# opendilab/DI-engine

Hardware: NVIDIA H100
Metric: learner transitions/sec (GAE+ppo_error fwd+bwd, T=128 x B=4096 per GPU) (higher is better)
Workload: dtype f32

## Files before the change

### di-engine_b200/csrc/gae_tile.cuh

```cuda
#pragma once
#include "common.cuh"

namespace b200rl {

template <int ID, int COUNT>
__device__ __forceinline__ void named_bar_sync() {
    asm volatile("bar.sync %0, %1;" ::"n"(ID), "n"(COUNT) : "memory");
}
template <int ID, int COUNT>
__device__ __forceinline__ void named_bar_arrive() {
    asm volatile("bar.arrive %0, %1;" ::"n"(ID), "n"(COUNT) : "memory");
}
template <int COUNT>
__device__ __forceinline__ void chunk_arrive(int k) {
    if (k == 0) named_bar_arrive<1, COUNT>();
    else if (k == 1) named_bar_arrive<2, COUNT>();
    else if (k == 2) named_bar_arrive<3, COUNT>();
    else named_bar_arrive<4, COUNT>();
}
__device__ __forceinline__ void scanned_arrive(int k) {
    if (k == 0) named_bar_arrive<5, 64>();
    else if (k == 1) named_bar_arrive<6, 64>();
    else if (k == 2) named_bar_arrive<7, 64>();
    else named_bar_arrive<8, 64>();
// ... 97 lines not shown
                        const long long c = c0 + cc;
                        if (r >= 0 && c < C) {
                            const long long off = (lo + r) * C + c;
                            const long long aoff = (lo + r) * Caux + c / A;
                            float nvv = next_value[off];
                            if (vscale != 0.f) nvv = fmul(nvv, vscale);
                            const float dnn = done ? done[aoff] : 0.f;
                            const float tff = traj ? traj[aoff] : dnn;
                            if (done) {
                                const float mm = fmul(nvv, fsub(1.f, dnn));
                                if (mask_inplace && dnn != 0.f) next_value[off] = mm;
                                nvv = mm;
                            }
                            const float vvv = vscale != 0.f ? fmul(value[off], vscale) : value[off];
                            s_d[k][rr][cc] = fsub(fadd(reward[aoff], fmul(gamma, nvv)), vvv);
                            s_f[k][rr][cc] = fmul(gl, fsub(1.f, tff));
                        }
                    }
                    chunk_arrive<NTHREADS>(k);
                }
            }
        } else {
            const int cc = threadIdx.x;
            const bool lane_ok = cc < TC && c0 + cc < C;
#pragma unroll 1
            for (int k = 0; k < GAE_NCHUNK; ++k) {
                chunk_wait<NTHREADS>(k);
                const int rtop = rows - 1 - k * GAE_CH;
                if (lane_ok && rtop >= 0) {
                    if (rtop >= GAE_CH - 1) {
                        float d[GAE_CH], f[GAE_CH];
#pragma unroll
                        for (int j = 0; j < GAE_CH; ++j) {
                            d[j] = s_d[k][j][cc];
                            f[j] = s_f[k][j][cc];
                        }
#pragma unroll
                        for (int j = 0; j < GAE_CH; ++j) {
                            carry = fadd(d[j], fmul(f[j], carry));
                            s_d[k][j][cc] = carry;
                        }
                    } else {
                        for (int j = 0; j <= rtop; ++j) {
                            carry = fadd(s_d[k][j][cc], fmul(s_f[k][j][cc], carry));
                            s_d[k][j][cc] = carry;
                        }
                    }
                }
                scanned_arrive(k);
            }
        }
        if (!is_scan) {
            constexpr int NLW = NL / 32;
            const int lw = ltid >> 5, ll = ltid & 31;
#pragma unroll 1
            for (int k = 0; k < GAE_NCHUNK; ++k) {
                if (k % NLW != lw) continue;
                scanned_wait(k);
                const int rtop = rows - 1 - k * GAE_CH;
                if (VEC) {
                    constexpr int TPR = TC / 4;
                    for (int i = ll; i < GAE_CH * TPR; i += 32) {
                        const int rr = i / TPR, cq = (i % TPR) * 4;
                        const int r = rtop - rr;
                        if (r >= 0 && c0 + cq < C) {
                            const float4 a4 = *reinterpret_cast<const float4*>(&s_d[k][rr][cq]);
                            stg_stream4(reinterpret_cast<float4*>(adv + (lo + r) * C + c0 + cq), a4);
                        }
                    }
                } else {
                    for (int i = ll; i < GAE_CH * TC; i += 32) {
                        const int rr = i / TC, cc = i % TC;
                        const int r = rtop - rr;
                        if (r >= 0 && c0 + cc < C) adv[(lo + r) * C + c0 + cc] = s_d[k][rr][cc];
                    }
                }
                on_chunk_done((T - hi) / GAE_CH + k, rtop >= 0);
            }
        }
        if (lo > 0) __syncthreads();
    }
}

}
```

### di-engine_b200/csrc/policy.cu

```cuda
#include <math.h>

#include "../../include/b200rl.h"
#include "policy_stats.cuh"

namespace b200rl {

constexpr int GS_NT = 1024;
constexpr int GS_MAX_T = 24576;

template <int VN>
__global__ void __launch_bounds__(GS_NT) gae_seq_kernel(const float* __restrict__ value, float* __restrict__ next_value,
                                                       const float* __restrict__ reward, const float* __restrict__ done,
                                                       const float* __restrict__ traj, float* __restrict__ adv, int T,
                                                       float gamma, float gl, int mask_inplace, RetArgs ra) {
    pdl_prologue();
    extern __shared__ float s_seq[];
    float* s_d = s_seq;
    float* s_f = s_seq + T;
    __shared__ int s_nseg;
    __shared__ int s_cnt[GS_NT / 32];
    const int tid = threadIdx.x;
    const float vs = ra.vscale;
    float mu = 0.f, sigma = 1.f;
    if constexpr (VN == VN_POPART) {
        mu = *ra.mu;
        sigma = *ra.sigma;
    }
    for (int t = tid; t < T; t += GS_NT) {
        const float v = vn_decode<VN>(value[t], vs);
        float nv = vn_decode<VN>(next_value[t], vs);
        float r = reward[t];
        if constexpr (VN == VN_POPART) r = __fdiv_rn(fsub(r, mu), sigma);
        const float d = done ? done[t] : 0.f;
        const float tf = traj ? traj[t] : d;
        if (done) {
            nv = fmul(nv, fsub(1.f, d));
            if (VN == VN_PPO && mask_inplace && d != 0.f) next_value[t] = nv;
        }
        s_d[t] = fsub(fadd(r, fmul(gamma, nv)), v);
        s_f[t] = fmul(gl, fsub(1.f, tf));
    }
    __syncthreads();
    const int strip = (T + GS_NT - 1) / GS_NT;
    const int t0 = tid * strip, t1 = min(T, t0 + strip);
    int mine = 0;
    for (int t = t0; t < t1; ++t) mine += (s_f[t] == 0.f || t == T - 1) ? 1 : 0;
    int incl = mine;
    const int lane = tid & 31, wid = tid >> 5;
#pragma unroll
    for (int o = 1; o < 32; o <<= 1) {
        const int n = __shfl_up_sync(0xffffffffu, incl, o);
        if (lane >= o) incl += n;
    }
    if (lane == 31) s_cnt[wid] = incl;
    __syncthreads();
    if (wid == 0) {
        int w = s_cnt[lane];
#pragma unroll
        for (int o = 1; o < 32; o <<= 1) {
            const int n = __shfl_up_sync(0xffffffffu, w, o);
            if (lane >= o) w += n;
        }
        s_cnt[lane] = w;
        if (lane == 31) s_nseg = w;
    }
    __syncthreads();
    const int base = incl - mine + (wid ? s_cnt[wid - 1] : 0);
    __shared__ int s_end[GS_NT];
    const int nseg = s_nseg;
    const bool fits = nseg <= GS_NT;
    if (fits) {
        int k = base;
        for (int t = t0; t < t1; ++t)
            if (s_f[t] == 0.f || t == T - 1) s_end[k++] = t;
    }
    __syncthreads();
    if (fits) {
        if (tid < nseg) {
            const int hi = s_end[tid];
            const int lo = tid ? s_end[tid - 1] + 1 : 0;
            float carry = 0.f;
            int t = hi;
            for (; t - 15 >= lo; t -= 16) {
                float d[16], f[16];
#pragma unroll
// ... 32 lines not shown
        if (cut >= 0) atomicMax(&s_cut, cut);
        __syncthreads();
        const int c = s_cut;
        for (int t = tid; t <= c; t += GS_NT) s_d[t] = __int_as_float(0x7fc00000);
        __syncthreads();
    }
    double acc[4] = {0.0, 0.0, 0.0, 0.0}, pv[2];
    ret_pivots<VN>(vs, vn_decode<VN>(ld_after_wait(value), vs), s_d[0], pv);
    for (int t = tid; t < T; t += GS_NT) {
        const float a = s_d[t];
        adv[t] = a;
        moments_add(acc[2], acc[3], a, pv[1]);
        if (ra.ret_unnorm || ra.value_out || ra.ret_out || ra.stats) {
            float ru, vo, ro;
            moments_add(acc[0], acc[1], ret_encode<VN>(vs, vn_decode<VN>(value[t], vs), a, ru, vo, ro), pv[0]);
            if (ra.ret_unnorm) ra.ret_unnorm[t] = ru;
            if (ra.value_out) ra.value_out[t] = vo;
            if (ra.ret_out) ra.ret_out[t] = ro;
        }
    }
    if (ra.stats || ra.adv_stats) {
        double tot[4];
        if (stats_grid_join<4, GS_NT>(acc, tot, nullptr, nullptr)) write_ret_stats<VN>(ra, tot, pv, (double)T);
    }
}

template <int VN, bool VEC>
__global__ void __launch_bounds__(256) returns_kernel(const float* __restrict__ value, const float* __restrict__ adv,
                                                      long long n, RetArgs ra, double* __restrict__ ws_part,
                                                      unsigned int* __restrict__ ws_join) {
    pdl_prologue();
    const float vs = ra.vscale;
    double acc[4] = {0.0, 0.0, 0.0, 0.0}, pv[2];
    const long long stride = (long long)gridDim.x * 256;
    long long i = (long long)blockIdx.x * 256 + threadIdx.x;
    if (VEC) {
        const long long n4 = n >> 2;
        const float4* v4 = reinterpret_cast<const float4*>(value);
        const float4* a4 = reinterpret_cast<const float4*>(adv);
        float4 v = make_float4(0.f, 0.f, 0.f, 0.f), a = v;
        if (i < n4) {
            v = v4[i];
            a = a4[i];
        }
        ret_pivots<VN>(vs, ret_value<VN>(ld_after_wait(value), vs), ld_after_wait(adv), pv);
        for (; i < n4; i += stride) {
            float4 ru, vo, ro;
            ret_one<VN>(vs, v.x, a.x, ru.x, vo.x, ro.x, acc, pv);
            ret_one<VN>(vs, v.y, a.y, ru.y, vo.y, ro.y, acc, pv);
            ret_one<VN>(vs, v.z, a.z, ru.z, vo.z, ro.z, acc, pv);
            ret_one<VN>(vs, v.w, a.w, ru.w, vo.w, ro.w, acc, pv);
            if (ra.ret_unnorm) reinterpret_cast<float4*>(ra.ret_unnorm)[i] = ru;
            if (ra.value_out) reinterpret_cast<float4*>(ra.value_out)[i] = vo;
            if (ra.ret_out) reinterpret_cast<float4*>(ra.ret_out)[i] = ro;
            if (i + stride < n4) {
                v = v4[i + stride];
                a = a4[i + stride];
            }
        }
    } else {
        float v = 0.f, a = 0.f;
        if (i < n) {
            v = value[i];
            a = adv[i];
        }
        ret_pivots<VN>(vs, ret_value<VN>(ld_after_wait(value), vs), ld_after_wait(adv), pv);
        for (; i < n; i += stride) {
            float ru, vo, ro;
            ret_one<VN>(vs, v, a, ru, vo, ro, acc, pv);
            if (ra.ret_unnorm) ra.ret_unnorm[i] = ru;
            if (ra.value_out) ra.value_out[i] = vo;
            if (ra.ret_out) ra.ret_out[i] = ro;
            if (i + stride < n) {
                v = value[i + stride];
                a = adv[i + stride];
            }
        }
    }
    if (!ra.stats && !ra.adv_stats) return;
    double tot[4];
    if (stats_grid_join<4, 256>(acc, tot, ws_part, ws_join)) write_ret_stats<VN>(ra, tot, pv, (double)n);
}

__global__ void __launch_bounds__(256) adv_stats_kernel(const float* __restrict__ x, long long n, float* __restrict__ out,
                                                        double* __restrict__ ws_part, unsigned int* __restrict__ ws_join) {
    pdl_prologue();
    const double p = stats_pivot(ld_after_wait(x));
    double acc[2] = {0.0, 0.0};
    for (long long i = (long long)blockIdx.x * 256 + threadIdx.x; i < n; i += (long long)gridDim.x * 256)
        moments_add(acc[0], acc[1], x[i], p);
    double tot[2];
    if (stats_grid_join<2, 256>(acc, tot, ws_part, ws_join)) write_adv_stats(out, tot[0], tot[1], p, (double)n);
}

__global__ void __launch_bounds__(256) normalize_kernel(const float* __restrict__ x, const float* __restrict__ stats,
                                                        long long n, float* __restrict__ out) {
    pdl_prologue();
    const float m = ld_after_wait(stats), d = ld_after_wait(stats + 1);
    for (long long i = (long long)blockIdx.x * 256 + threadIdx.x; i < n; i += (long long)gridDim.x * 256)
        out[i] = __fdiv_rn(fsub(x[i], m), d);
}

__global__ void __launch_bounds__(256) impala_mask_kernel(const float* __restrict__ values, const float* __restrict__ rewards,
                                                          const float* __restrict__ done, long long T, long long B,
                                                          float* __restrict__ values_out, float* __restrict__ rewards_out,
                                                          float* __restrict__ weights_out) {
    pdl_prologue();
    const long long n = (T + 1) * B;
    for (long long i = (long long)blockIdx.x * 256 + threadIdx.x; i < n; i += (long long)gridDim.x * 256) {
        const long long t = i / B;
        const float m = t >= 1 ? fsub(1.f, done[i - B]) : 1.f;
        values_out[i] = t >= 1 ? fmul(values[i], m) : values[i];
        if (t < T) {
            if (weights_out) weights_out[i] = m;
            if (rewards_out) rewards_out[i] = fmul(rewards[i], m);
        }
    }
}

enum ValueMap : int { VM_SYMLOG = 0, VM_INV_SYMLOG = 1, VM_H_INV = 2, VM_POPART_REWARD = 3 };

template <int M>
__device__ __forceinline__ float value_map(float x, float mu, float sigma) {
    if constexpr (M == VM_SYMLOG) return vn_symlog(x);
    else if constexpr (M == VM_INV_SYMLOG) return vn_inv_symlog(x);
    else if constexpr (M == VM_H_INV) return vn_h_inv(x);
    else return __fdiv_rn(fsub(x, mu), sigma);
}

template <int M>
__global__ void __launch_bounds__(256) value_map_kernel(const float* __restrict__ x0, float* __restrict__ y0,
                                                        const float* __restrict__ x1, float* __restrict__ y1, long long n,
                                                        const float* __restrict__ mu, const float* __restrict__ sigma) {
    pdl_prologue();
    float m = 0.f, sg = 1.f;
    if constexpr (M == VM_POPART_REWARD) {
        m = *mu;
        sg = *sigma;
    }
    for (long long i = (long long)blockIdx.x * 256 + threadIdx.x; i < n; i += (long long)gridDim.x * 256) {
        y0[i] = value_map<M>(x0[i], m, sg);
        if (x1) y1[i] = value_map<M>(x1[i], m, sg);
    }
}

template <int M>
__global__ void __launch_bounds__(256) value_map_bwd_kernel(const float* __restrict__ x, const float* __restrict__ g,
                                                            float* __restrict__ dx, long long n) {
    pdl_prologue();
    for (long long i = (long long)blockIdx.x * 256 + threadIdx.x; i < n; i += (long long)gridDim.x * 256) {
        const float xi = x[i], s = vn_sign(xi), gs = fmul(g[i], s);
        const float d = M == VM_SYMLOG ? __fdiv_rn(gs, fadd(fabsf(xi), 1.f)) : fmul(gs, expf(fabsf(xi)));
        dx[i] = fadd(0.f, fmul(d, s));
    }
}

}

using namespace b200rl;

namespace b200rl {
int gae_scan(const float* value, float* next_value, const float* reward, const float* done, const float* traj_flag, float* adv,
             long long T, long long C, long long A, double gamma_d, double lambda_d, int mask_next_value_inplace,
             float vscale, void* stream);
}

static double* ws_stats_part(float* ws) { return reinterpret_cast<double*>(ws + WS_CTRL_WORDS); }
static unsigned int* ws_joins(float* ws) { return reinterpret_cast<unsigned int*>(ws + WS_FX_OFF_WORDS + 48); }
static_assert(WS_CTRL_WORDS % 2 == 0 && WS_CTRL_WORDS + NUM_SMS * 8 * 4 * 2 <= WS_PARTIAL_LIMIT_WORDS,
              "the statistics rows fit the workspace's partial region");

extern "C" int b200rl_adv_stats(const float* x, long long n, float* stats2, float* workspace, size_t workspace_bytes,
                                void* stream) {
    if (!x || !stats2 || !workspace || n < 1 || workspace_bytes < WS_MIN_BYTES) return B200RL_ERR_ARG;
    long long grid = div_up(n, 256 * 8);
    if (grid > NUM_SMS * 4) grid = NUM_SMS * 4;
    if (grid < 1) grid = 1;
    return launch_k(adv_stats_kernel, (int)grid, 256, 0, (cudaStream_t)stream, x, n, stats2, ws_stats_part(workspace),
                    ws_joins(workspace));
}

extern "C" int b200rl_normalize(const float* x, const float* stats2, long long n, float* out, void* stream) {
    if (!x || !stats2 || !out || n < 0) return B200RL_ERR_ARG;
    if (n == 0) return B200RL_OK;
    long long grid = div_up(n, 256 * 4);
    if (grid > NUM_SMS * 8) grid = NUM_SMS * 8;
    return launch_k(normalize_kernel, (int)grid, 256, 0, (cudaStream_t)stream, x, stats2, n, out);
}

extern "C" int b200rl_gae_returns(const float* value, float* next_value, const float* reward, const float* done,
                                  const float* traj_flag, long long T, long long C, long long A, double gamma,
                                  double lambda_, int mask_next_value_inplace, double value_scale, float* adv,
                                  float* unnormalized_return, float* value_out, float* return_out, float* stats3,
                                  float* adv_stats2, float* workspace, size_t workspace_bytes, void* stream) {
    if (T < 1 || C < 1 || A < 1 || !value || !next_value || !reward || !adv || !workspace ||
        workspace_bytes < WS_MIN_BYTES || value_scale < 0.0)
        return B200RL_ERR_ARG;
    RetArgs ra{};
    ra.vscale = (float)value_scale;
    ra.ret_unnorm = unnormalized_return; ra.value_out = value_out; ra.ret_out = return_out; ra.stats = stats3;
    ra.adv_stats = adv_stats2;
    cudaStream_t st = (cudaStream_t)stream;
    if (C == 1 && T <= GS_MAX_T) {
        const size_t smem = (size_t)2 * T * sizeof(float);
        if (int rc = smem_opt_in<gae_seq_kernel<VN_PPO>>(smem)) return rc;
        return launch_k(gae_seq_kernel<VN_PPO>, 1, GS_NT, smem, st, value, next_value, reward, done, traj_flag, adv, (int)T,
                        (float)gamma, (float)(gamma * lambda_), mask_next_value_inplace, ra);
    }
    const bool want_epi = unnormalized_return || value_out || return_out || stats3 || adv_stats2;
    int rc = gae_scan(value, next_value, reward, done, traj_flag, adv, T, C, A, gamma, lambda_, mask_next_value_inplace,
                      (float)value_scale, stream);
    if (rc != 0 || !want_epi) return rc;
    const long long n = T * C;
    const bool vec = (n % 4 == 0) && aligned16(value) && aligned16(adv) && (!unnormalized_return || aligned16(unnormalized_return)) &&
                     (!value_out || aligned16(value_out)) && (!return_out || aligned16(return_out));
    long long grid = div_up(n, 256 * (vec ? 8 : 4));
    if (grid > NUM_SMS * 8) grid = NUM_SMS * 8;
    if (vec)
        return launch_k(returns_kernel<VN_PPO, true>, (int)grid, 256, 0, st, value, (const float*)adv, n, ra,
                        ws_stats_part(workspace), ws_joins(workspace));
    return launch_k(returns_kernel<VN_PPO, false>, (int)grid, 256, 0, st, value, (const float*)adv, n, ra,
                    ws_stats_part(workspace), ws_joins(workspace));
}

static long long map_grid(long long n) {
    long long grid = div_up(n, 256 * 4);
    if (grid > NUM_SMS * 8) grid = NUM_SMS * 8;
    return grid < 1 ? 1 : grid;
}

template <int VN>
static int launch_gae_seq(const float* value, const float* next_value, const float* reward, const float* done,
                          const float* traj_flag, float* adv, long long T, double gamma, double lambda_, const RetArgs& ra,
                          cudaStream_t st) {
    const size_t smem = (size_t)2 * T * sizeof(float);
    if (int rc = smem_opt_in<gae_seq_kernel<VN>>(smem)) return rc;
    return launch_k(gae_seq_kernel<VN>, 1, GS_NT, smem, st, value, const_cast<float*>(next_value), reward, done, traj_flag,
                    adv, (int)T, (float)gamma, (float)(gamma * lambda_), 0, ra);
}

template <int VN>
static int launch_returns(const float* value, const float* adv, long long n, const RetArgs& ra, float* workspace,
                          cudaStream_t st) {
    const bool vec = (n % 4 == 0) && aligned16(value) && aligned16(adv) && (!ra.value_out || aligned16(ra.value_out)) &&
                     (!ra.ret_out || aligned16(ra.ret_out));
    long long grid = div_up(n, 256 * (vec ? 8 : 4));
    if (grid > NUM_SMS * 8) grid = NUM_SMS * 8;
    if (vec)
        return launch_k(returns_kernel<VN, true>, (int)grid, 256, 0, st, value, adv, n, ra, ws_stats_part(workspace),
                        ws_joins(workspace));
    return launch_k(returns_kernel<VN, false>, (int)grid, 256, 0, st, value, adv, n, ra, ws_stats_part(workspace),
                    ws_joins(workspace));
}

template <int VN>
static int launch_gae_returns_tc(const float* value, const float* next_value, const float* reward, const float* done,
                                 const float* traj_flag, float* adv, long long T, long long C, double gamma, double lambda_,
                                 const RetArgs& ra, float* scratch, float* workspace, cudaStream_t st) {
    const long long n = T * C;
    const float* v = value;
    const float* nv = next_value;
    const float* r = reward;
    int rc = 0;
    if constexpr (VN == VN_RESCALE || VN == VN_SYMLOG) {
        constexpr int M = VN == VN_RESCALE ? VM_H_INV : VM_INV_SYMLOG;
        rc = launch_k(value_map_kernel<M>, (int)map_grid(n), 256, 0, st, value, scratch, next_value, scratch + n, n,
                      (const float*)nullptr, (const float*)nullptr);
        v = scratch;
        nv = scratch + n;
    } else if constexpr (VN == VN_POPART) {
        rc = launch_k(value_map_kernel<VM_POPART_REWARD>, (int)map_grid(n), 256, 0, st, reward, scratch,
                      (const float*)nullptr, (float*)nullptr, n, ra.mu, ra.sigma);
        r = scratch;
    }
    if (rc) return rc;
    rc = gae_scan(v, const_cast<float*>(nv), r, done, traj_flag, adv, T, C, 1, gamma, lambda_, 0,
                  VN == VN_BASELINE ? ra.vscale : 0.f, st);
    if (rc || !(ra.value_out || ra.ret_out || ra.stats || ra.adv_stats)) return rc;
    return launch_returns<VN>(v, adv, n, ra, workspace, st);
}

template <int VN>
static int gae_returns_norm(const float* value, const float* next_value, const float* reward, const float* done,
                            const float* traj_flag, float* adv, long long T, long long C, double gamma, double lambda_,
                            const RetArgs& ra, float* scratch, float* workspace, cudaStream_t st) {
    if (C == 1 && T <= GS_MAX_T)
        return launch_gae_seq<VN>(value, next_value, reward, done, traj_flag, adv, T, gamma, lambda_, ra, st);
    return launch_gae_returns_tc<VN>(value, next_value, reward, done, traj_flag, adv, T, C, gamma, lambda_, ra, scratch,
                                     workspace, st);
}

extern "C" int b200rl_gae_returns_norm(const float* value, const float* next_value, const float* reward, const float* done,
// ... 64 lines not shown
```

### di-engine_b200/csrc/policy_stats.cuh

```cuda
#pragma once
#include <math.h>

#include "common.cuh"

namespace b200rl {

template <class T>
__device__ __forceinline__ T warp_sum_t(T v) {
#pragma unroll
    for (int o = 16; o > 0; o >>= 1) v += __shfl_xor_sync(0xffffffffu, v, o);
    return v;
}

template <int K, int NT>
__device__ __forceinline__ void block_sum_d(double (&v)[K], double (&tot)[K]) {
    __shared__ double s_bs[K][NT / 32];
    const int lane = threadIdx.x & 31, wid = threadIdx.x >> 5;
#pragma unroll
    for (int k = 0; k < K; ++k) {
        const double r = warp_sum_t(v[k]);
        if (lane == 0) s_bs[k][wid] = r;
    }
    __syncthreads();
    if (threadIdx.x == 0) {
// ... 7 lines not shown
    __syncthreads();
}

struct RetArgs {
    float vscale;
    float* ret_unnorm;
    float* value_out;
    float* ret_out;
    float* stats;
    float* adv_stats;
    const float* mu;
    const float* sigma;
};

enum ValueNorm : int { VN_BASELINE = 0, VN_RESCALE = 1, VN_SYMLOG = 2, VN_POPART = 3, VN_PPO = 4 };

__device__ __forceinline__ float vn_sign(float x) { return (float)((0.f < x) - (x < 0.f)); }

__device__ __forceinline__ float vn_h(float x) {
    return fadd(fmul(vn_sign(x), fsub(__fsqrt_rn(fadd(fabsf(x), 1.f)), 1.f)), fmul(0.01f, x));
}
__device__ __forceinline__ float vn_h_inv(float x) {
    const float u = __fdiv_rn(fsub(__fsqrt_rn(fadd(1.f, fmul(0.04f, fadd(fadd(fabsf(x), 1.f), 0.01f)))), 1.f), 0.02f);
    return fmul(vn_sign(x), fsub(fmul(u, u), 1.f));
}
__device__ __forceinline__ float vn_symlog(float x) { return fmul(vn_sign(x), logf(fadd(fabsf(x), 1.f))); }
__device__ __forceinline__ float vn_inv_symlog(float x) { return fmul(vn_sign(x), fsub(expf(fabsf(x)), 1.f)); }

template <int VN>
__device__ __forceinline__ float vn_decode(float v, float vs) {
    if constexpr (VN == VN_PPO || VN == VN_BASELINE) return vs != 0.f ? fmul(v, vs) : v;
    else if constexpr (VN == VN_RESCALE) return vn_h_inv(v);
    else if constexpr (VN == VN_SYMLOG) return vn_inv_symlog(v);
    else return v;
}

template <int VN>
__device__ __forceinline__ float vn_encode(float v, float vs) {
    if constexpr (VN == VN_PPO || VN == VN_BASELINE) return vs != 0.f ? __fdiv_rn(v, vs) : v;
    else if constexpr (VN == VN_RESCALE) return vn_h(v);
    else if constexpr (VN == VN_SYMLOG) return vn_symlog(v);
    else return v;
}

template <int VN>
__device__ __forceinline__ float ret_encode(float vs, float v, float a, float& ru, float& vo, float& ro) {
    const float r = fadd(v, a);
    ru = r;
    vo = vn_encode<VN>(v, vs);
    ro = vn_encode<VN>(r, vs);
    return VN == VN_PPO ? r : ro;
}

__device__ __forceinline__ double stats_pivot(float x0) { return isfinite(x0) ? (double)x0 : 0.0; }

__device__ __forceinline__ float ld_after_wait(const float* p) { return __ldcg(p); }

__device__ __forceinline__ void moments_add(double& s1, double& s2, float x, double p) {
    const double d = (double)x - p;
    s1 += d;
    s2 = fma(d, d, s2);
}

template <int VN>
__device__ __forceinline__ float ret_value(float v, float vs) {
    if constexpr (VN == VN_PPO || VN == VN_BASELINE) return vn_decode<VN>(v, vs);
    else return v;
}

template <int VN>
__device__ __forceinline__ void ret_one(float vs, float v, float a, float& ru, float& vo, float& ro, double (&acc)[4],
                                        const double (&pv)[2]) {
    moments_add(acc[0], acc[1], ret_encode<VN>(vs, ret_value<VN>(v, vs), a, ru, vo, ro), pv[0]);
    moments_add(acc[2], acc[3], a, pv[1]);
}

template <int VN>
__device__ __forceinline__ void ret_pivots(float vs, float v0, float a0, double (&pv)[2]) {
    float ru, vo, ro;
    pv[0] = stats_pivot(ret_encode<VN>(vs, v0, a0, ru, vo, ro));
    pv[1] = stats_pivot(a0);
}

template <int K, int NT>
__device__ __forceinline__ bool stats_grid_join(double (&acc)[K], double (&tot)[K], double* part, unsigned int* ticket) {
    __shared__ bool s_last;
    block_sum_d<K, NT>(acc, tot);
    if (gridDim.x == 1) return threadIdx.x == 0;
    if (threadIdx.x == 0) {
#pragma unroll
        for (int k = 0; k < K; ++k) part[(size_t)blockIdx.x * K + k] = tot[k];
        __threadfence();
        s_last = atomicAdd(ticket, 1u) == gridDim.x - 1;
    }
    __syncthreads();
    if (!s_last) return false;
    __threadfence();
    double v[K];
#pragma unroll
    for (int k = 0; k < K; ++k) v[k] = 0.0;
    for (unsigned int b = threadIdx.x; b < gridDim.x; b += NT)
#pragma unroll
        for (int k = 0; k < K; ++k) v[k] += __ldcg(part + (size_t)b * K + k);
    block_sum_d<K, NT>(v, tot);
    if (threadIdx.x == 0) *ticket = 0u;
    return threadIdx.x == 0;
}

__device__ __forceinline__ void write_adv_stats(float* out, double s1, double s2, double p, double nn) {
    const double d = s1 / nn;
    const double var = (s2 - s1 * d) / (nn - 1.0);
    const double sd = var != var ? var : sqrt(fmax(var, 0.0));
    out[0] = (float)(p + d);
    out[1] = fadd((float)sd, 1e-8f);
}

template <int VN>
__device__ __forceinline__ double pop_var(double v) {
    return (VN != VN_PPO && v != v) ? v : fmax(v, 0.0);
}

template <int VN>
__device__ __forceinline__ void write_ret_stats(const RetArgs& ra, const double (&tot)[4], const double (&pv)[2],
                                                double nn) {
    if (ra.stats) {
        const double d = tot[0] / nn;
        ra.stats[0] = (float)(pv[0] + d);
        ra.stats[1] = (float)pop_var<VN>(tot[1] / nn - d * d);
        ra.stats[2] = (float)nn;
    }
    if (ra.adv_stats) write_adv_stats(ra.adv_stats, tot[2], tot[3], pv[1], nn);
}

}
```

### di-engine_b200/csrc/ppo.cu

```cuda
#include "../../include/b200rl.h"
#include "ppo_math.cuh"

namespace b200rl {

template <int NC, int WHAT>
__global__ void __launch_bounds__(PPO_THREADS) ppo_tile_kernel(PpoArgs a, float* out, float* ws) {
    constexpr int PPO_R = PPO_CT;
    pdl_prologue();
    extern __shared__ __align__(128) unsigned char smem[];
    constexpr bool GRADS = (WHAT != PPO_FWD);
    constexpr bool LOSSES = (WHAT != PPO_BWD);
    const int N = NC ? NC : a.N;
    const int tid = threadIdx.x;
    const int wid = tid >> 5, lane = tid & 31;
    const bool is_producer = wid == PPO_CW;
    const bool has_pre = a.logit_pre != nullptr, has_w = a.weight != nullptr;
    const PpoTileLayout L = ppo_layout(N, has_pre, has_w, PPO_R);
    const int warp_out_bytes = 32 * N * 4;
    unsigned char* outbuf = smem + PPO_STAGES * L.stage_bytes;
    uint64_t* full = reinterpret_cast<uint64_t*>(outbuf + (GRADS ? PPO_OUTBUFS * L.logit_bytes : 0));
    uint64_t* empty = full + PPO_STAGES;

    float g[4] = {0.f, 0.f, 0.f, 0.f};
    if (GRADS && upstream<4>(a.rec, WHAT == PPO_BWD, ppo_owned(a), g)) return;
// ... 184 lines not shown
        ratio_s /= (float)G;
    }
    for (int g = 0; g < G; ++g) {
        const float* rn = zn + (size_t)g * N;
        const float* ro = zo + (size_t)g * N;
        float* gr = gz + (size_t)g * N;
        const int act = (int)a.action[s * G + g];
        float lse_n, ent;
        row_lse_entropy<L>([&](int j) { return rn[j]; }, N, lane, lse_n, ent);
        const float lse_o = row_lse<L>([&](int j) { return ro[j]; }, N, lane);
        const float lp_n = rn[act] - lse_n;
        const float ratio_g = expf(lp_n - (ro[act] - lse_o));
        if (G == 1) ratio_s = ratio_g;
        float dsel;
        surrogate(ratio_s, adv, a.clip_lo, a.clip_hi, a.dual_clip, dsel, false, a.factor ? a.factor[s] : 1.f);
        float c_act = g_pol * (-w * inv_s) * dsel * ratio_g / (float)G;
        if (zp) {
            const float* rp = zp + (size_t)g * N;
            const float lse_p = row_lse<L>([&](int j) { return rp[j]; }, N, lane);
            float dk;
            kl_term(lp_n - (rp[act] - lse_p), a.kl_type, dk);
            c_act += g_kl * dk * inv_m;
        }
        const float c_ent = g_ent * w * inv_m;
        for (int j = lane; j < N; j += L) {
            const float lp = fmaxf(rn[j] - lse_n, kF32Min);
            const float p = expf(lp);
            float gj = -c_act * p - c_ent * p * (lp + ent);
            if (j == act) gj += c_act;
            gr[j] = gj;
        }
    }
    if (lane == 0) {
        float dterm;
        value_term(a.value_new[s], a.value_old[s], a.ret[s], a.clip, a.use_value_clip, dterm);
        a.grad_value[s] = g_val * 0.5f * w * inv_s * dterm;
    }
    }
}

static bool tile_path_ok(const PpoArgs& a) {
    const bool al = aligned16(a.logit_new) && aligned16(a.logit_old) && (!a.logit_pre || aligned16(a.logit_pre)) &&
                    aligned16(a.action) && aligned16(a.value_new) && aligned16(a.value_old) && aligned16(a.adv) &&
                    aligned16(a.ret) && (!a.weight || aligned16(a.weight)) &&
                    (!a.grad_logit || aligned16(a.grad_logit));
    return a.G == 1 && a.N <= 32 && al;
}

template <int NT>
__global__ void __launch_bounds__(NT) ppo_value_kernel(const float* __restrict__ value_new,
                                                       const float* __restrict__ value_old,
                                                       const float* __restrict__ ret, const float* __restrict__ weight,
                                                       long long S, float clip, int use_clip, float* __restrict__ out,
                                                       float* __restrict__ dvalue, float* ws) {
    pdl_prologue();
    float acc[1] = {0.f};
    const float inv_s = 1.f / (float)S;
    for (long long i = (long long)blockIdx.x * NT + threadIdx.x; i < S; i += (long long)gridDim.x * NT) {
        const float w = weight ? weight[i] : 1.f;
        float d;
        const float t = value_term(value_new[i], use_clip ? value_old[i] : 0.f, ret[i], clip, use_clip, d);
        acc[0] += t * w;
        if (dvalue) dvalue[i] = 0.5f * w * inv_s * d;
    }
    double tot[1];
    if (grid_sum<1, NT>(acc, tot, ws, 0) && threadIdx.x == 0) out[0] = (float)(0.5 * tot[0] / (double)S);
}

template <int NC, int WHAT>
static int launch_tile(const PpoArgs& a, float* out, float* ws, size_t ws_bytes, cudaStream_t st) {
    constexpr int PPO_R = PPO_CT;
    const PpoTileLayout L = ppo_layout(a.N, a.logit_pre != nullptr, a.weight != nullptr, PPO_R);
    const size_t smem = (size_t)PPO_STAGES * L.stage_bytes + (WHAT != PPO_FWD ? (size_t)PPO_OUTBUFS * L.logit_bytes : 0) +
                        2 * PPO_STAGES * sizeof(uint64_t);
    constexpr auto kern = ppo_tile_kernel<NC, WHAT>;
    if (smem > 227 * 1024) return B200RL_ERR_ARG;
    int sm_count, per_sm;
    if (int rc = resident_ctas<kern>(PPO_THREADS, smem, sm_count, per_sm)) return rc;
    if (per_sm > 6) per_sm = 6;
    const long long n_tiles = (a.S + PPO_R - 1) / PPO_R;
    long long grid = (long long)sm_count * ((WHAT == PPO_BWD && a.rec.used) ? 1 : per_sm);
    if (grid > n_tiles) grid = n_tiles;
    if (WHAT != PPO_BWD && !ws_partials_fit((long long)(grid * 6), ws_bytes)) return B200RL_ERR_WORKSPACE;
    if (int rc = launch_k(kern, (int)grid, PPO_THREADS, smem, st, a, out, ws)) return rc;
    if (WHAT == PPO_BWD) return B200RL_OK;
    return launch_finalize(ws, out, ppo_finalize_args(a.S, a.logit_pre != nullptr, (int)grid), st);
}

template <int WHAT>
static int dispatch_tile(const PpoArgs& a, float* out, float* ws, size_t ws_bytes, cudaStream_t st) {
    return with_nc(a.N, [&](auto nc) { return launch_tile<nc, WHAT>(a, out, ws, ws_bytes, st); });
}

}

using namespace b200rl;

static int fill_args(PpoArgs& a, const float* logit_new, const float* logit_old, const float* logit_pretrained,
                     const long long* action, const float* value_new, const float* value_old, const float* adv,
                     const float* return_, const float* weight, long long S, long long G, long long N,
                     double clip_ratio, int use_value_clip, double dual_clip, int kl_type, const float* adv_stats,
                     const float* factor) {
    a.adv_stats = adv_stats;
    a.factor = factor;
    a.logit_new = logit_new; a.logit_old = logit_old; a.logit_pre = logit_pretrained; a.action = action;
    a.value_new = value_new; a.value_old = value_old; a.adv = adv; a.ret = return_; a.weight = weight;
    a.S = S; a.G = (int)G; a.N = (int)N; a.clip = (float)clip_ratio; a.clip_lo = (float)(1.0 - clip_ratio);
    a.clip_hi = (float)(1.0 + clip_ratio); a.dual_clip = (float)dual_clip;
    a.use_value_clip = use_value_clip; a.kl_type = kl_type;
    if (S < 0 || G < 1 || N < 1) return B200RL_ERR_ARG;
    if (!logit_new || !logit_old || !action || !value_new || !value_old || !adv || !return_) return B200RL_ERR_ARG;
    if (kl_type < 1 || kl_type > 3) return B200RL_ERR_ARG;
    return B200RL_OK;
}

extern "C" int b200rl_ppo_fwd(const float* logit_new, const float* logit_old, const float* logit_pretrained,
                              const long long* action, const float* value_new, const float* value_old,
                              const float* adv, const float* return_, const float* weight, long long S, long long G,
                              long long N, double clip_ratio, int use_value_clip, double dual_clip, int kl_type,
                              const float* adv_stats, const float* factor, float* out, float* workspace,
                              size_t workspace_bytes, void* stream) {
    PpoArgs a{};
    int rc = fill_args(a, logit_new, logit_old, logit_pretrained, action, value_new, value_old, adv, return_, weight,
                       S, G, N, clip_ratio, use_value_clip, dual_clip, kl_type, adv_stats, factor);
    if (rc != B200RL_OK || !out || !workspace) return rc != B200RL_OK ? rc : B200RL_ERR_ARG;
    if (S == 0) return B200RL_ERR_ARG;
    cudaStream_t st = (cudaStream_t)stream;
    if (tile_path_ok(a)) return dispatch_tile<PPO_FWD>(a, out, workspace, workspace_bytes, st);
    constexpr int NT = 128;
    const bool warp = a.N > 64;
    int grid = warp ? div_up(S, NT / 32) : div_up(S, NT);
    if (grid > NUM_SMS * 16) grid = NUM_SMS * 16;
    if (!ws_partials_fit((long long)((size_t)grid * 6), workspace_bytes)) return B200RL_ERR_WORKSPACE;
    if (warp) return launch_k(ppo_fwd_kernel<NT, 2>, grid, NT, 0, st, a, out, workspace);
    return launch_k(ppo_fwd_kernel<NT, 1>, grid, NT, 0, st, a, out, workspace);
}

extern "C" int b200rl_ppo_fwd_grad(const float* logit_new, const float* logit_old, const float* logit_pretrained,
                                   const long long* action, const float* value_new, const float* value_old,
                                   const float* adv, const float* return_, const float* weight, long long S,
                                   long long G, long long N, double clip_ratio, int use_value_clip, double dual_clip,
                                   int kl_type, const float* adv_stats, const float* factor, const float* g_expected,
                                   float* g_used, float* out,
                                   float* grad_logit_new, float* grad_value_new, float* workspace,
                                   size_t workspace_bytes, void* stream) {
    PpoArgs a{};
    int rc = fill_args(a, logit_new, logit_old, logit_pretrained, action, value_new, value_old, adv, return_, weight,
                       S, G, N, clip_ratio, use_value_clip, dual_clip, kl_type, adv_stats, factor);
    if (rc != B200RL_OK) return rc;
    if (!workspace || S == 0 || !upstream_args_ok(0, out, true, grad_logit_new && grad_value_new, g_expected, g_used))
        return B200RL_ERR_ARG;
    a.rec = forward_record(g_expected, g_used); a.grad_logit = grad_logit_new; a.grad_value = grad_value_new;
    if (!tile_path_ok(a)) return B200RL_ERR_ARG;
    return dispatch_tile<PPO_FWD_GRAD>(a, out, workspace, workspace_bytes, (cudaStream_t)stream);
}

extern "C" int b200rl_ppo_fused_supported(const float* logit_new, const float* logit_old,
                                          const float* logit_pretrained, const long long* action,
                                          const float* value_new, const float* value_old, const float* adv,
                                          const float* return_, const float* weight, const float* grad_logit_new,
                                          long long G, long long N) {
    PpoArgs a{};
    a.logit_new = logit_new; a.logit_old = logit_old; a.logit_pre = logit_pretrained; a.action = action;
    a.value_new = value_new; a.value_old = value_old; a.adv = adv; a.ret = return_; a.weight = weight;
    a.grad_logit = const_cast<float*>(grad_logit_new); a.G = (int)G; a.N = (int)N;
    return tile_path_ok(a) ? 1 : 0;
}

extern "C" int b200rl_ppo_bwd(const float* logit_new, const float* logit_old, const float* logit_pretrained,
// ... 46 lines not shown
```

Before: 21.34 billion.

## Add warp-specialized fused GAE scan and returns epilogue kernel with deferred PDL wait

Adds a single warp-specialized kernel for the GAE returns path. One producer warp streams value/next_value/reward/done/traj tiles into an 8-stage shared-memory ring with cp.async and mbarriers. One warp computes deltas and runs the backward scan per column tile, and eight epilogue warps write advantages, returns and running moment statistics. This replaces the separate scan kernel plus epilogue/stats passes, removing extra global round trips and launches. It also adds dependency-chain tracking so the grid-dependency wait can be deferred when inputs don't alias prior writes. The cost is a single warp doing the serial scan per CTA, plus extra pivot-shift logic in the grid join.

```diff
diff --git a/di-engine_b200/csrc/gae_tile.cuh b/di-engine_b200/csrc/gae_tile.cuh
--- a/di-engine_b200/csrc/gae_tile.cuh
+++ b/di-engine_b200/csrc/gae_tile.cuh
@@ -203,4 +203,79 @@
     }
 }
 
-}
+
+template <int TC, int R>
+__device__ __forceinline__ void cw_delta_f(const float* raw, float (*ab)[TC], float (*fb)[TC], long long t0, long long c0,
+                                           long long B, bool has_done, bool has_traj, float gamma, float gl, float vscale,
+                                           bool mask_inplace, float* next_value, int lane) {
+    constexpr int PR = TC / 4;
+    const float* rv = raw;
+    const float* rn = rv + R * TC;
+    const float* rr = rn + R * TC;
+    const float* rd = rr + R * TC;
+    const float* rt = rd + R * TC;
+    const int cq = (lane % PR) * 4;
+#pragma unroll
+    for (int p = 0; p < R * PR / 32; ++p) {
+        const int jj = p * (32 / PR) + lane / PR;
+        const long long t = t0 + jj;
+        if (t >= 0 && c0 + cq < B) {
+            const int o = jj * TC + cq;
+            const float4 v4 = *reinterpret_cast<const float4*>(rv + o);
+            const float4 n4 = *reinterpret_cast<const float4*>(rn + o);
+            const float4 r4 = *reinterpret_cast<const float4*>(rr + o);
+            const float4 d4 = has_done ? *reinterpret_cast<const float4*>(rd + o) : make_float4(0.f, 0.f, 0.f, 0.f);
+            const float4 t4 = has_traj ? *reinterpret_cast<const float4*>(rt + o) : d4;
+            float vv[4] = {v4.x, v4.y, v4.z, v4.w}, nn[4] = {n4.x, n4.y, n4.z, n4.w};
+            float rw[4] = {r4.x, r4.y, r4.z, r4.w}, dd[4] = {d4.x, d4.y, d4.z, d4.w};
+            float tt[4] = {t4.x, t4.y, t4.z, t4.w};
+            float de[4], fa[4];
+            bool changed = false;
+#pragma unroll
+            for (int k = 0; k < 4; ++k) {
+                if (vscale != 0.f) {
+                    vv[k] = fmul(vv[k], vscale);
+                    nn[k] = fmul(nn[k], vscale);
+                }
+                if (has_done) {
+                    changed |= (dd[k] != 0.f);
+                    nn[k] = fmul(nn[k], fsub(1.f, dd[k]));
+                }
+                de[k] = fsub(fadd(rw[k], fmul(gamma, nn[k])), vv[k]);
+                fa[k] = fmul(gl, fsub(1.f, tt[k]));
+            }
+            *reinterpret_cast<float4*>(&ab[jj][cq]) = make_float4(de[0], de[1], de[2], de[3]);
+            *reinterpret_cast<float4*>(&fb[jj][cq]) = make_float4(fa[0], fa[1], fa[2], fa[3]);
+            if (changed && mask_inplace)
+                *reinterpret_cast<float4*>(next_value + t * B + c0 + cq) = make_float4(nn[0], nn[1], nn[2], nn[3]);
+        }
+    }
+}
+
+template <int TC, int R>
+__device__ __forceinline__ float cw_scan(float (*ab)[TC], const float (*fb)[TC], long long t0, long long c0, long long B,
+                                         float carry, int lane) {
+    if (lane < TC && c0 + lane < B) {
+        if (t0 >= 0) {
+            float d[R], g[R];
+#pragma unroll
+            for (int k = 0; k < R; ++k) {
+                d[k] = ab[R - 1 - k][lane];
+                g[k] = fb[R - 1 - k][lane];
+            }
+#pragma unroll
+            for (int k = 0; k < R; ++k) {
+                carry = fadd(d[k], fmul(g[k], carry));
+                ab[R - 1 - k][lane] = carry;
+            }
+        } else {
+            for (int jj = R - 1; jj >= 0 && t0 + jj >= 0; --jj) {
+                carry = fadd(ab[jj][lane], fmul(fb[jj][lane], carry));
+                ab[jj][lane] = carry;
+            }
+        }
+    }
+    return carry;
+}
+
+}
diff --git a/di-engine_b200/csrc/policy.cu b/di-engine_b200/csrc/policy.cu
--- a/di-engine_b200/csrc/policy.cu
+++ b/di-engine_b200/csrc/policy.cu
@@ -1,6 +1,7 @@
 #include <math.h>
 
 #include "../../include/b200rl.h"
+#include "gae_tile.cuh"
 #include "policy_stats.cuh"
 
 namespace b200rl {
@@ -199,6 +200,184 @@
     if (stats_grid_join<4, 256>(acc, tot, ws_part, ws_join)) write_ret_stats<VN>(ra, tot, pv, (double)n);
 }
 
+constexpr int RW_TC = 32;
+constexpr int RW_R = 8;
+constexpr int RW_EW = 8;
+constexpr int RW_THREADS = RW_EW * 32 + 64;
+constexpr int RW_ARR = RW_R * RW_TC;
+constexpr int RW_STAGE_FLOATS = 6 * RW_ARR;
+constexpr int RW_STAGES = 8;
+constexpr int RW_STATS = 9;
+static_assert(RW_EW * 32 == RW_ARR, "one epilogue thread per transition of a chunk");
+
+struct RwArgs {
+    const float* value;
+    float* next_value;
+    const float* reward;
+    const float* done;
+    const float* traj;
+    float* adv;
+    long long T, B;
+    float gamma, gl;
+    int mask_inplace;
+    int defer_wait;
+    RetArgs ra;
+    double* part;
+    unsigned int* ticket;
+};
+
+__global__ void __launch_bounds__(RW_THREADS, 1) gae_returns_ws_kernel(RwArgs g) {
+    extern __shared__ __align__(128) float rw_smem[];
+    float (*fbuf)[RW_TC] = reinterpret_cast<float (*)[RW_TC]>(rw_smem + RW_STAGES * RW_STAGE_FLOATS);
+    uint64_t* full = reinterpret_cast<uint64_t*>(rw_smem + RW_STAGES * RW_STAGE_FLOATS + RW_ARR);
+    uint64_t* adv_ready = full + RW_STAGES;
+    uint64_t* done = full + 2 * RW_STAGES;
+    __shared__ double s_p0[2];
+    const int tid = threadIdx.x, wid = tid >> 5, lane = tid & 31;
+    const long long T = g.T, B = g.B;
+    const long long n_tiles = (B + RW_TC - 1) / RW_TC, n_chunks = (T + RW_R - 1) / RW_R;
+    const bool has_done = g.done != nullptr, has_traj = g.traj != nullptr;
+    const float vs = g.ra.vscale;
+    if (tid == 0) {
+        for (int s = 0; s < RW_STAGES; ++s) {
+            mbar_init(&full[s], 32);
+            mbar_init(&adv_ready[s], 1);
+            mbar_init(&done[s], RW_EW);
+        }
+        mbar_fence_init();
+        s_p0[0] = s_p0[1] = 0.0;
+    }
+    auto dep_wait = [] {
+        asm volatile("griddepcontrol.wait;" ::: "memory");
+        asm volatile("griddepcontrol.launch_dependents;" ::: "memory");
+    };
+    if (!g.defer_wait) dep_wait();
+    __syncthreads();
+
+    long long tile = blockIdx.x, q = 0;
+    auto next = [&] {
+        if (++q >= n_chunks) {
+            q = 0;
+            tile += gridDim.x;
+        }
+    };
+    double acc[RW_STATS];
+#pragma unroll
+    for (int k = 0; k < RW_STATS; ++k) acc[k] = 0.0;
+
+    if (wid == RW_EW) {
+        const float* src[5] = {g.value, g.next_value, g.reward, g.done, g.traj};
+        int s = 0, ph = 0;
+        for (int j = 0; tile < n_tiles; ++j) {
+            if (j >= RW_STAGES) mbar_wait(&done[s], (uint32_t)(ph ^ 1));
+            const long long c0 = tile * RW_TC, t0 = T - (q + 1) * RW_R;
+            const int W4 = (int)((B - c0) < RW_TC ? (B - c0) : RW_TC) / 4;
+            float* st = rw_smem + s * RW_STAGE_FLOATS;
+#pragma unroll
+            for (int a = 0; a < 5; ++a) {
+                if (!src[a]) continue;
+#pragma unroll
+                for (int k = 0; k < RW_ARR / 4 / 32; ++k) {
+                    const int p = lane + 32 * k, row = p / (RW_TC / 4), o = p % (RW_TC / 4);
+                    if (t0 + row >= 0 && o < W4) cpa16(st + a * RW_ARR + p * 4, src[a] + (t0 + row) * B + c0 + o * 4);
+                }
+            }
+            cpa_mbar_arrive(&full[s]);
+            if (++s == RW_STAGES) { s = 0; ph ^= 1; }
+            next();
+        }
+    } else if (wid == RW_EW + 1) {
+        if (g.defer_wait) dep_wait();
+        float carry = 0.f;
+        int s = 0, ph = 0;
+        for (int j = 0; tile < n_tiles; ++j) {
+            const long long c0 = tile * RW_TC, t0 = T - (q + 1) * RW_R;
+            if (q == 0) carry = 0.f;
+            float* st = rw_smem + s * RW_STAGE_FLOATS;
+            float (*ab)[RW_TC] = reinterpret_cast<float (*)[RW_TC]>(st + 5 * RW_ARR);
+            mbar_wait(&full[s], (uint32_t)ph);
+            cw_delta_f<RW_TC, RW_R>(st, ab, fbuf, t0, c0, B, has_done, has_traj, g.gamma, g.gl, vs, g.mask_inplace != 0,
+                                    g.next_value, lane);
+            __syncwarp();
+            carry = cw_scan<RW_TC, RW_R>(ab, fbuf, t0, c0, B, carry, lane);
+            __syncwarp();
+            if (lane == 0) mbar_arrive(&adv_ready[s]);
+            if (++s == RW_STAGES) { s = 0; ph ^= 1; }
+            next();
+        }
+    } else {
+        if (g.defer_wait) dep_wait();
+        const RetArgs& ra = g.ra;
+        const int jj = tid / RW_TC, c = tid % RW_TC;
+        double pq[2] = {0.0, 0.0};
+        int s = 0, ph = 0;
+        for (int j = 0; tile < n_tiles; ++j) {
+            const long long c0 = tile * RW_TC, t = T - (q + 1) * RW_R + jj;
+            const float* st = rw_smem + s * RW_STAGE_FLOATS;
+            const float (*ab)[RW_TC] = reinterpret_cast<const float (*)[RW_TC]>(st + 5 * RW_ARR);
+            mbar_wait(&full[s], (uint32_t)ph);
+            mbar_wait(&adv_ready[s], (uint32_t)ph);
+            if (j == 0) ret_pivots<VN_PPO>(vs, vn_decode<VN_PPO>(st[(RW_R - 1) * RW_TC], vs), ab[RW_R - 1][0], pq);
+            if (t >= 0 && c0 + c < B) {
+                const long long i = t * B + c0 + c;
+                const float v = vn_decode<VN_PPO>(st[jj * RW_TC + c], vs), a = ab[jj][c];
+                float ru, vo, ro;
+                const float r = ret_encode<VN_PPO>(vs, v, a, ru, vo, ro);
+                __stcs(g.adv + i, a);
+                if (ra.ret_unnorm) __stcs(ra.ret_unnorm + i, ru);
+                if (ra.value_out) __stcs(ra.value_out + i, vo);
+                if (ra.ret_out) __stcs(ra.ret_out + i, ro);
+                moments_add(acc[0], acc[1], r, pq[0]);
+                moments_add(acc[2], acc[3], a, pq[1]);
+                acc[4] += 1.0;
+                if (i == 0) {
+                    double p0[2];
+                    ret_pivots<VN_PPO>(vs, v, a, p0);
+                    s_p0[0] = p0[0];
+                    s_p0[1] = p0[1];
+                }
+            }
+            __syncwarp();
+            if (lane == 0) mbar_arrive(&done[s]);
+            if (++s == RW_STAGES) { s = 0; ph ^= 1; }
+            next();
+        }
+        if (tid == 0) {
+            acc[5] = pq[0];
+            acc[6] = pq[1];
+        }
+    }
+    if (!g.ra.stats && !g.ra.adv_stats) return;
+    __syncthreads();
+    if (tid == 0 && blockIdx.x == 0) {
+        acc[7] = s_p0[0];
+        acc[8] = s_p0[1];
+    }
+    auto move = [](double (&v)[RW_STATS], const double (&r)[RW_STATS], double p0, double p1) {
+        double s1 = r[0], s2 = r[1], a1 = r[2], a2 = r[3];
+        moments_move(s1, s2, r[4], r[5], p0);
+        moments_move(a1, a2, r[4], r[6], p1);
+        v[0] += s1; v[1] += s2; v[2] += a1; v[3] += a2; v[4] += r[4];
+    };
+    double* part = g.part;
+    double tot[RW_STATS];
+    const bool last = stats_grid_join<RW_STATS, RW_THREADS>(
+        acc, tot, part, g.ticket,
+        [&](double (&v)[RW_STATS], const double (&r)[RW_STATS]) { move(v, r, __ldcg(part + 7), __ldcg(part + 8)); });
+    if (!last) return;
+    double pv[2] = {tot[7], tot[8]};
+    if (gridDim.x == 1) {
+        double v[RW_STATS] = {0.0, 0.0, 0.0, 0.0, 0.0, 0.0, 0.0, 0.0, 0.0};
+        move(v, tot, pv[0], pv[1]);
+        for (int k = 0; k < 5; ++k) tot[k] = v[k];
+    } else {
+        pv[0] = __ldcg(part + 7);
+        pv[1] = __ldcg(part + 8);
+    }
+    const double t4[4] = {tot[0], tot[1], tot[2], tot[3]};
+    write_ret_stats<VN_PPO>(g.ra, t4, pv, (double)T * (double)B);
+}
+
 __global__ void __launch_bounds__(256) adv_stats_kernel(const float* __restrict__ x, long long n, float* __restrict__ out,
                                                         double* __restrict__ ws_part, unsigned int* __restrict__ ws_join) {
     pdl_prologue();
@@ -303,6 +482,43 @@
     long long grid = div_up(n, 256 * 4);
     if (grid > NUM_SMS * 8) grid = NUM_SMS * 8;
     return launch_k(normalize_kernel, (int)grid, 256, 0, (cudaStream_t)stream, x, stats2, n, out);
+}
+
+static int launch_gae_returns_ws(const float* value, float* next_value, const float* reward, const float* done,
+                                 const float* traj_flag, float* adv, long long T, long long B, double gamma, double lambda_,
+                                 int mask_inplace, const RetArgs& ra, float* workspace, size_t workspace_bytes,
+                                 cudaStream_t st) {
+    RwArgs g{};
+    g.value = value; g.next_value = next_value; g.reward = reward; g.done = done; g.traj = traj_flag; g.adv = adv;
+    g.T = T; g.B = B;
+    g.gamma = (float)gamma; g.gl = (float)(gamma * lambda_);
+    g.mask_inplace = mask_inplace && done;
+    g.ra = ra;
+    g.part = ws_stats_part(workspace);
+    g.ticket = ws_joins(workspace);
+    const size_t smem = (size_t)(RW_STAGES * RW_STAGE_FLOATS + RW_ARR) * sizeof(float) + 3 * RW_STAGES * sizeof(uint64_t);
+    int sm_count, per_sm;
+    if (int rc = resident_ctas<gae_returns_ws_kernel>(RW_THREADS, smem, sm_count, per_sm)) return rc;
+    const long long n_tiles = (B + RW_TC - 1) / RW_TC;
+    long long grid = (long long)sm_count * per_sm;
+    if (grid > n_tiles) grid = n_tiles;
+    if (!ws_partials_fit(grid * RW_STATS * 2, workspace_bytes)) return B200RL_ERR_WORKSPACE;
+    const ChainPoint at = capture_now(st);
+    const long long F = T * B * 4;
+    ByteSpan span[8] = {byte_span(value, F), byte_span(next_value, F), byte_span(reward, F), byte_span(done, F),
+                        byte_span(traj_flag, F)};
+    g.defer_wait = chain_may_defer(st, at, span, 5);
+    if (int rc = launch_k(gae_returns_ws_kernel, (int)grid, RW_THREADS, smem, st, g)) return rc;
+    const ByteSpan w[] = {byte_span(adv, F),
+                          byte_span(ra.ret_unnorm, F),
+                          byte_span(ra.value_out, F),
+                          byte_span(ra.ret_out, F),
+                          byte_span(ra.stats, 3 * sizeof(float)),
+                          byte_span(ra.adv_stats, 2 * sizeof(float)),
+                          byte_span(workspace, (long long)workspace_bytes),
+                          byte_span(g.mask_inplace ? next_value : nullptr, F)};
+    chain_report(st, at, true, w, (int)(sizeof(w) / sizeof(w[0])));
+    return B200RL_OK;
 }
 
 extern "C" int b200rl_gae_returns(const float* value, float* next_value, const float* reward, const float* done,
@@ -325,6 +541,10 @@
                         (float)gamma, (float)(gamma * lambda_), mask_next_value_inplace, ra);
     }
     const bool want_epi = unnormalized_return || value_out || return_out || stats3 || adv_stats2;
+    if (want_epi && A == 1 && C > 1 && C % 4 == 0 && aligned16(value) && aligned16(next_value) && aligned16(reward) &&
+        (!done || aligned16(done)) && (!traj_flag || aligned16(traj_flag)))
+        return launch_gae_returns_ws(value, next_value, reward, done, traj_flag, adv, T, C, gamma, lambda_,
+                                     mask_next_value_inplace, ra, workspace, workspace_bytes, st);
     int rc = gae_scan(value, next_value, reward, done, traj_flag, adv, T, C, A, gamma, lambda_, mask_next_value_inplace,
                       (float)value_scale, stream);
     if (rc != 0 || !want_epi) return rc;
diff --git a/di-engine_b200/csrc/policy_stats.cuh b/di-engine_b200/csrc/policy_stats.cuh
--- a/di-engine_b200/csrc/policy_stats.cuh
+++ b/di-engine_b200/csrc/policy_stats.cuh
@@ -113,8 +113,17 @@
     pv[1] = stats_pivot(a0);
 }
 
-template <int K, int NT>
-__device__ __forceinline__ bool stats_grid_join(double (&acc)[K], double (&tot)[K], double* part, unsigned int* ticket) {
+struct RowSum {
+    template <int K>
+    __device__ __forceinline__ void operator()(double (&v)[K], const double (&r)[K]) const {
+#pragma unroll
+        for (int k = 0; k < K; ++k) v[k] += r[k];
+    }
+};
+
+template <int K, int NT, class AddRow = RowSum>
+__device__ __forceinline__ bool stats_grid_join(double (&acc)[K], double (&tot)[K], double* part, unsigned int* ticket,
+                                                AddRow add_row = AddRow()) {
     __shared__ bool s_last;
     block_sum_d<K, NT>(acc, tot);
     if (gridDim.x == 1) return threadIdx.x == 0;
@@ -130,12 +139,22 @@
     double v[K];
 #pragma unroll
     for (int k = 0; k < K; ++k) v[k] = 0.0;
-    for (unsigned int b = threadIdx.x; b < gridDim.x; b += NT)
+    for (unsigned int b = threadIdx.x; b < gridDim.x; b += NT) {
+        double r[K];
 #pragma unroll
-        for (int k = 0; k < K; ++k) v[k] += __ldcg(part + (size_t)b * K + k);
+        for (int k = 0; k < K; ++k) r[k] = __ldcg(part + (size_t)b * K + k);
+        add_row(v, r);
+    }
     block_sum_d<K, NT>(v, tot);
     if (threadIdx.x == 0) *ticket = 0u;
     return threadIdx.x == 0;
+}
+
+__device__ __forceinline__ void moments_move(double& s1, double& s2, double n, double q, double p) {
+    const double d = q - p;
+    if (d == 0.0) return;
+    s2 = s2 + 2.0 * d * s1 + n * d * d;
+    s1 = s1 + n * d;
 }
 
 __device__ __forceinline__ void write_adv_stats(float* out, double s1, double s2, double p, double nn) {
diff --git a/di-engine_b200/csrc/ppo.cu b/di-engine_b200/csrc/ppo.cu
--- a/di-engine_b200/csrc/ppo.cu
+++ b/di-engine_b200/csrc/ppo.cu
@@ -290,9 +290,17 @@
     long long grid = (long long)sm_count * ((WHAT == PPO_BWD && a.rec.used) ? 1 : per_sm);
     if (grid > n_tiles) grid = n_tiles;
     if (WHAT != PPO_BWD && !ws_partials_fit((long long)(grid * 6), ws_bytes)) return B200RL_ERR_WORKSPACE;
+    const ChainPoint at = WHAT == PPO_FWD_GRAD ? capture_now(st) : ChainPoint{};
     if (int rc = launch_k(kern, (int)grid, PPO_THREADS, smem, st, a, out, ws)) return rc;
     if (WHAT == PPO_BWD) return B200RL_OK;
-    return launch_finalize(ws, out, ppo_finalize_args(a.S, a.logit_pre != nullptr, (int)grid), st);
+    if (int rc = launch_finalize(ws, out, ppo_finalize_args(a.S, a.logit_pre != nullptr, (int)grid), st)) return rc;
+    if (WHAT == PPO_FWD_GRAD) {
+        const ByteSpan w[] = {byte_span(a.grad_logit, a.S * a.G * a.N * 4), byte_span(a.grad_value, a.S * 4),
+                              byte_span(a.rec.used, 4 * sizeof(float)), byte_span(ws, (long long)ws_bytes),
+                              byte_span(out, 8 * sizeof(float))};
+        chain_report(st, at, false, w, 5);
+    }
+    return B200RL_OK;
 }
 
 template <int WHAT>
```

New measurement: 21.34 billion (median of 6 runs). Within noise of the previous version (+0.0%).
